# ynotstartups/implisolid

Hardware: AMD Instinct MI355X
Metric: Mvoxels/s (eval+MC) at 256^3 & 512^3 (higher is better)
Workload: dtype f32; 1 GPU; config4: seeded ~20-node MP5 CSG tree with twist/union/difference (scenes.config4, seed 20251015), box [-1,1]^3, R=512, eval+MC, mesh resident in HBM; resolution=512, voxels=134217728, samples=135005697, cells=135796744, verts=360248, faces=720496, program_instr=42, tree_depth=8, parallelism=zslab1, voxels_per_rank=134217728

## Files before the change

### implisolid_amd/csrc/abi.hip

```cpp
#include <chrono>
#include <cmath>
#include <cstdio>
#include <cstdlib>
#include <cstring>
#include <ctime>
#include <map>
#include <memory>
#include <string>
#include <vector>
#include <thread>
#include <mutex>
#include <algorithm>
#include <functional>

#include "../../include/implisolid.h"
#include "engine.hpp"
#include "batch_device.hpp"
#include "brick_modes.hpp"
#include "jit.hpp"

#include <chrono>
#include <rocprofiler-sdk-roctx/roctx.h>
#include "host.hpp"
#include "ob02.hpp"
// ... 1381 lines not shown
#define SLAB_TRY(expr)                                 \
    try {                                              \
        expr;                                          \
    } catch (const std::exception& e) {                \
        report(e.what(), false);                       \
        return -1;                                     \
    }                                                  \
    return 0;

int implisolid_slab_eval(implisolid_slab* s, void* stream) { SLAB_TRY(s->engine.eval_field((hipStream_t)stream)) }
int implisolid_slab_count(implisolid_slab* s, void* stream) { SLAB_TRY(s->engine.count((hipStream_t)stream)) }
int implisolid_slab_emit(implisolid_slab* s, const uint32_t* d_offsets, void* stream) {
    SLAB_TRY(s->engine.emit(d_offsets, (hipStream_t)stream))
}
int implisolid_slab_emit_verts(implisolid_slab* s, void* stream) {
    SLAB_TRY(s->engine.emit_verts((hipStream_t)stream))
}
int implisolid_slab_emit_faces(implisolid_slab* s, const uint32_t* d_offsets, const uint32_t* d_gathered, int rank,
                               void* stream) {
    SLAB_TRY(s->engine.emit_faces(d_offsets, d_gathered, rank, (hipStream_t)stream))
}
const uint32_t* implisolid_slab_counters(implisolid_slab* s) { return s->engine.d_counters(); }
int implisolid_slab_counts(implisolid_slab* s, void* stream, uint32_t out[3]) {
    try {
        bool of = false;
        SlabCounts c = s->engine.read_counts((hipStream_t)stream, &of);
        const bool grew = s->engine.ensure_capacity(c);
        out[0] = c.n_verts();
        out[1] = c.n_faces();
        out[2] = (of || grew) ? 1u : 0u;
    } catch (const std::exception& e) {
        report(e.what(), false);
        return -1;
    }
    return 0;
}
int implisolid_slab_grid(implisolid_slab* s, int32_t out[8]) {
    const GridDesc& g = s->engine.grid();
    const int32_t v[8] = {g.R, g.res, g.cz0, g.cz1, g.cz_emit, g.fz0, g.fz1, s->engine.depth()};
    std::memcpy(out, v, sizeof v);
    return 0;
}
int implisolid_slab_copy_counts(implisolid_slab* s, uint32_t* d_dst, void* stream) {
    SLAB_TRY(IMPLI_HIP(hipMemcpyAsync(d_dst, s->engine.d_counters() + 2, 4 * sizeof(uint32_t), hipMemcpyDeviceToDevice,
                                      (hipStream_t)stream)))
}
int implisolid_slab_copy_mesh(implisolid_slab* s, float* d_verts, int32_t* d_faces, int64_t nv, int64_t nf, void* stream) {
    SLAB_TRY(
        if (nv > 0) IMPLI_HIP(hipMemcpyAsync(d_verts, s->engine.d_verts(), (size_t)nv * 12, hipMemcpyDeviceToDevice, (hipStream_t)stream));
        if (nf > 0) IMPLI_HIP(hipMemcpyAsync(d_faces, s->engine.d_faces(), (size_t)nf * 12, hipMemcpyDeviceToDevice, (hipStream_t)stream)))
}
int implisolid_slab_set_offsets(implisolid_slab* s, uint32_t voff, uint32_t foff) {
    SLAB_TRY(s->engine.set_offsets(voff, foff))
}
int implisolid_slab_download(implisolid_slab* s, float* verts, int32_t* faces, void* stream) {
    try {
        bool of = false;
        const SlabCounts c = s->engine.read_counts((hipStream_t)stream, &of);
        if (of) throw HipError("slab output overflowed; call implisolid_slab_counts and emit again");
        s->engine.download(verts, faces, c, (hipStream_t)stream);
    } catch (const std::exception& e) {
        report(e.what(), false);
        return -1;
    }
    return 0;
}
int implisolid_slab_emit_normals(implisolid_slab* s, void* stream) { SLAB_TRY(s->engine.emit_normals((hipStream_t)stream)) }
float* implisolid_slab_normals(implisolid_slab* s) { return s->engine.d_normals(); }
int implisolid_slab_download_normals(implisolid_slab* s, float* out, void* stream) {
    try {
        const SlabCounts c = s->engine.read_counts((hipStream_t)stream, nullptr);
        s->engine.download_normals(out, c, (hipStream_t)stream);
    } catch (const std::exception& e) {
        report(e.what(), false);
        return -1;
    }
    return 0;
}
float* implisolid_slab_verts(implisolid_slab* s) { return s->engine.d_verts(); }
int32_t* implisolid_slab_faces(implisolid_slab* s) { return s->engine.d_faces(); }
float* implisolid_slab_field(implisolid_slab* s) { return s->engine.d_field(); }

int implisolid_slab_stats_n(implisolid_slab* s, int64_t* out, int n) {
    constexpr int kStats = 10;
    try {
        if (!out || n < 0) throw InputError("slab_stats: null output or negative length");
        uint32_t c[16];
        s->engine.raw_counters(c, 0);
        const GridDesc& g = s->engine.grid();
        const int64_t v[kStats] = {
            n_units(g),
            c[6],
            c[2], c[3], c[4], c[5],
            g.n_cells,
            c[14],
            c[1],
            c[0]};
        for (int k = 0; k < n && k < kStats; ++k) out[k] = v[k];
        return kStats;
    } catch (const std::exception& e) {
        report(e.what(), false);
        return -1;
    }
}

int implisolid_slab_stats(implisolid_slab* s, int64_t out[8]) {
    return implisolid_slab_stats_n(s, out, 8) < 0 ? -1 : 0;
}

int implisolid_slab_used_jit(implisolid_slab* s) { return s->engine.used_baked() ? 2 : s->engine.used_jit() ? 1 : 0; }
void implisolid_set_jit(int mode) { TreeJit::instance().set_mode(mode); }
void implisolid_set_jit_bake(int mode) { TreeJit::instance().set_bake(mode); }
void implisolid_jit_wait(void) { TreeJit::instance().wait_idle(); }
void implisolid_jit_stats(int32_t out[4], double* compile_seconds) {
    TreeJit& j = TreeJit::instance();
    out[0] = j.mode();
    out[1] = j.bake();
    out[2] = j.compiled();
    out[3] = j.disk_hits();
    if (compile_seconds) *compile_seconds = j.compile_seconds();
}
void implisolid_set_jit_max_modules(int n) { TreeJit::instance().set_max_modules(n); }
void implisolid_jit_modules(int32_t out[3]) {
    TreeJit& j = TreeJit::instance();
    out[0] = j.modules();
    out[1] = j.max_modules();
    out[2] = j.evicted();
}

int implisolid_slab_set_timing(implisolid_slab* s, int on) { SLAB_TRY(s->engine.set_timing(on != 0)) }
int implisolid_slab_kernel_times(implisolid_slab* s, float ms[6]) { SLAB_TRY(s->engine.kernel_times(ms)) }
int implisolid_slab_kernel_times_each(implisolid_slab* s, float ms[8]) { SLAB_TRY(s->engine.kernel_times_each(ms)) }

int64_t implisolid_slab_read_signs(implisolid_slab* s, uint8_t* out, int64_t capacity) {
    try {
        const GridDesc& g = s->engine.grid();
        const int64_t rows = (int64_t)g.n * (g.fz1 - g.fz0), rw = sign_row_words(g);
        const int64_t n = rows * g.n;
        if (out) {
            if (capacity < n) throw InputError("implisolid_slab_read_signs: buffer too small");
            std::vector<uint64_t> w((size_t)(rows * rw));
            IMPLI_HIP(hipDeviceSynchronize());
            IMPLI_HIP(hipMemcpy(w.data(), s->engine.d_signs(), w.size() * sizeof(uint64_t), hipMemcpyDeviceToHost));
            for (int64_t r = 0; r < rows; ++r)
                for (int x = 0; x < g.n; ++x) out[r * g.n + x] = (uint8_t)((w[(size_t)(r * rw + x / 64)] >> (x % 64)) & 1u);
        }
        return n;
    } catch (const std::exception& e) {
        report(e.what(), false);
        return -1;
    }
}

int implisolid_slab_brick_stats(implisolid_slab* s, int64_t out[3]) {
    try {
        s->engine.brick_stats(out, 0);
    } catch (const std::exception& e) {
        report(e.what(), false);
        return -1;
    }
    return 0;
}

int64_t implisolid_slab_read_field(implisolid_slab* s, float* out, int64_t capacity) {
    try {
        const GridDesc& g = s->engine.grid();
        const int64_t n = (int64_t)g.n * g.n * (int64_t)(g.fz1 - g.fz0);
        if (out) {
            if (capacity < n) throw InputError("implisolid_slab_read_field: buffer too small");
            IMPLI_HIP(hipDeviceSynchronize());
            std::vector<float> raw((size_t)field_samples(g));
            if (!raw.empty())
                IMPLI_HIP(hipMemcpy(raw.data(), s->engine.d_field(), raw.size() * sizeof(float), hipMemcpyDeviceToHost));
            const int layers = g.fz1 - g.fz0;
            for (int l = 0; l < layers; ++l)
                for (int y = 0; y < g.n; ++y)
                    for (int x = 0; x < g.n; ++x)
                        out[((int64_t)l * g.n + y) * g.n + x] = raw[(size_t)field_index(g, x, y, l)];
        }
// ... 585 lines not shown
```

### implisolid_amd/csrc/mc.hip

```cpp
#include <algorithm>
#include <cstdlib>
#include <stdexcept>

#include "eval_bricks.hpp"
#include "ifunc_device.hpp"
#include "kernels.hpp"
#include "mc_device.hpp"
#include "batch_device.hpp"

namespace impli {

GridDesc make_grid(int R, const float box[6], int cz0, int cz1, int cz_emit) {
    GridDesc g{};
    g.R = R;
    g.res = R + 5;
    g.n = R + 3;
    g.m = R + 2;
    for (int a = 0; a < 3; ++a) {
        const float width = box[2 * a + 1] - box[2 * a];
        g.w[a] = width / (float)R;
        g.lo[a] = box[2 * a];
        g.i0[a] = box[2 * a] / g.w[a] - 2.f;
    }
    g.cz0 = cz0;
// ... 12 lines not shown
        int n = 0;
        for (; s[n]; ++n) c.tri[n] = (uint8_t)((s[n] <= '9') ? s[n] - '0' : s[n] - 'a' + 10);
        c.ntri = (uint8_t)(n / 3);
        c.rank[0] = c.rank[1] = c.rank[2] = -1;
        int r = 0;
        for (int k = 0; k < n; ++k) {
            const int e = c.tri[k];
            const int slot = (e == 5) ? 0 : (e == 6) ? 1 : (e == 10) ? 2 : -1;
            if (slot >= 0 && c.rank[slot] < 0) c.rank[slot] = (int8_t)r++;
        }
        c.nown = (uint8_t)r;
        static const int owner_of_edge[12] = {5, 4, 4, 6, 2, 0, 0, 1, 3, 2, 0, 1};
        for (int k = 0; k < n; ++k) c.owners = (uint8_t)(c.owners | (1u << owner_of_edge[c.tri[k]]));
        auto neg = [ci](int k) { return (ci >> k) & 1; };
        const int crossing = (neg(5) ^ neg(6)) + (neg(6) ^ neg(7)) + (neg(2) ^ neg(6));
        int ec = 0, ei = 0, v = 0, ff = 0, opp = 0;
        for (const auto& e : kCubeEdges) { ec += neg(e[0]) ^ neg(e[1]); ei += neg(e[0]) & neg(e[1]); }
        for (int k = 0; k < 8; ++k) v += neg(k);
        for (const auto& f : kCubeFaces) ff += neg(f[0]) & neg(f[1]) & neg(f[2]) & neg(f[3]);
        for (const auto& o : kCubeOpposite) opp += (v == 6 && !neg(o[0]) && !neg(o[1])) ? 1 : 0;
        const int ntri_formula = (ci == 0 || ci == 255) ? 0 : ec - 2 * (v - ei + ff + 2 * opp);
        if (crossing != c.nown || (c.ntri > 0) != (ci != 0 && ci != 255) || ntri_formula != c.ntri)
            throw std::runtime_error("marching cubes: case table violates the count kernel's assumptions");
        out[ci] = c;
    }
}

namespace {

__device__ __forceinline__ uint32_t wave_sum(uint32_t x) {
#pragma unroll
    for (int o = 32; o > 0; o >>= 1) x += __shfl_xor(x, o, 64);
    return x;
}

__device__ __forceinline__ void mc_count_body(const GridDesc& g, const MCBuffers& b) {
    __shared__ uint32_t s_u[kGroupUnits][4];
    __shared__ uint32_t s_cm[kGroupUnits];
    __shared__ uint16_t s_fp[kGroupUnits * kMaxChunks];
    __shared__ uint32_t s_nf;
    const int t = threadIdx.x, nt_ = blockDim.x;
    for (int k = t; k < 4 * kGroupUnits; k += nt_) (&s_u[0][0])[k] = 0u;
    for (int k = t; k < kGroupUnits; k += nt_) s_cm[k] = 0u;
    if (t == 0) s_nf = 0u;
    const int64_t G = blockIdx.x;
    const int nch = n_chunks(g);
    const int64_t rows = n_rows(g), nu = n_units(g);
    const int64_t row0 = G * kGroupUnits * kUnitRows;
    __syncthreads();
    for (int p0 = 0; p0 < kGroupUnits * nch; p0 += nt_) {
        const int p = p0 + t, ui = p / nch, c = p - ui * nch;
        const int64_t u = G * kGroupUnits + ui;
        const bool cand = p < kGroupUnits * nch && u < nu && (!b.umark || b.umark[u * nch + c] == b.mark_id);
        const uint64_t m = __ballot(cand);
        uint32_t base = 0;
        if ((t & 63) == 0 && m) base = atomicAdd(&s_nf, (uint32_t)__popcll((unsigned long long)m));
        base = __shfl(base, 0, 64);
        if (cand) s_fp[base + __popcll((unsigned long long)(m & ((1ull << (t & 63)) - 1ull)))] = (uint16_t)(ui * kMaxChunks + c);
    }
    __syncthreads();
    const int n_items = (int)s_nf * kUnitRows;
    for (int i = t; i < n_items; i += nt_) {
        ChunkBits k;
        const uint32_t pr = s_fp[i / kUnitRows];
        const int ui = (int)(pr / kMaxChunks), c = (int)(pr % kMaxChunks);
        const int rb = ui * kUnitRows + i % kUnitRows;
        const bool ok = row0 + rb < rows;
        load_chunk(g, b.signs, ok ? row0 + rb : 0, c, k);
        if (!ok) k.nt = 0;
        if (!k.nt) continue;
        if (c < kChunkMaskBits) atomicOr(&s_cm[ui], 1u << c);
        const unsigned own = (unsigned)(__popcll((unsigned long long)((k.t01 ^ k.t11) & k.nt)) +
                                        __popcll((unsigned long long)((k.s11 ^ k.t11) & k.nt)) +
                                        __popcll((unsigned long long)((k.t10 ^ k.t11) & k.nt)));
        unsigned tri = 0, act = 0, hal = 0;
        if (k.z >= g.cz_emit) {
            act = (unsigned)__popcll((unsigned long long)k.nt);
            tri = chunk_triangles(k);
        } else {
            hal = own;
        }
        uint32_t* d = s_u[ui];
        if (own) atomicAdd(&d[0], own);
        if (tri) { atomicAdd(&d[1], tri); atomicAdd(&d[2], act); }
        if (hal) atomicAdd(&d[3], hal);
    }
    __syncthreads();
    if (t < 64) {
        const int64_t u = G * kGroupUnits + t;
        const uint32_t own = s_u[t][0], tri = s_u[t][1], act = s_u[t][2], hal = s_u[t][3];
        const bool ne = u < nu && (own | tri) != 0;
        const uint32_t eo = wave_incl_scan<uint32_t>(own, t) - own;
        const uint32_t et = wave_incl_scan<uint32_t>(tri, t) - tri;
        const uint32_t ea = wave_incl_scan<uint32_t>(act, t) - act;
        const uint64_t m = __ballot(ne);
        const uint32_t pos = (uint32_t)__popcll((unsigned long long)(m & ((1ull << t) - 1ull)));
        const uint32_t parts = ne ? min((uint32_t)kMaxParts, max(1u, (act + kPartCells - 1) / kPartCells)) : 0u;
        const bool heavy = act > kHeavyCells;
        const uint32_t ph = heavy ? parts : 0u, pl = heavy ? 0u : parts;
        const uint32_t eph = wave_incl_scan<uint32_t>(ph, t) - ph, epl = wave_incl_scan<uint32_t>(pl, t) - pl;
        if (ne) {
            b.unit_cnt[G * kGroupUnits + pos] = make_uint4((uint32_t)t, eo, et, ea);
            b.unit_part[G * kGroupUnits + pos] = (heavy ? eph : epl) | (parts << 16) | ((uint32_t)heavy << 20);
            b.unit_cmask[G * kGroupUnits + pos] = s_cm[t];
        }
        const uint32_t sums[kScanParts + 1] = {__shfl(eo + own, 63, 64), __shfl(et + tri, 63, 64),
                                               __shfl(ea + act, 63, 64), wave_sum(hal), __shfl(eph + ph, 63, 64),
                                               __shfl(epl + pl, 63, 64), (uint32_t)__popcll((unsigned long long)m)};
        if (t <= kScanParts) {
            const uint32_t v = t == 0 ? sums[0] : t == 1 ? sums[1] : t == 2 ? sums[2] : t == 3 ? sums[3]
                             : t == 4 ? sums[4] : t == 5 ? sums[5] : sums[6];
            b.scan_blk[(int64_t)t * gridDim.x + G] = v;
        }
    }
}
__global__ __launch_bounds__(512) void k_mc_count(GridDesc g, MCBuffers b) { mc_count_body(g, b); }

constexpr int kScanBlock = 256;
constexpr int kScanRows = kScanParts + 1;
template <int BS = kScanBlock>
__device__ __forceinline__ void unit_scan_body(const GridDesc& g, const MCBuffers& b) {
    static_assert(BS >= kGroupUnits, "a lane per unit of the group");
    __shared__ uint32_t s_part[BS / 64][kScanRows];
    __shared__ uint32_t s_base[kScanRows];
    const int64_t G = blockIdx.x, ng = n_groups(g);
    const int t = threadIdx.x, lane = t & 63, wid = t >> 6;
    const bool last = G == ng - 1;
    const uint32_t nne = b.scan_blk[kScanParts * ng + G];
    if (nne == 0 && !last) return;
    const uint4 e = b.unit_cnt[G * kGroupUnits + (t < (int)nne ? t : 0)];
    const uint32_t pp = b.unit_part[G * kGroupUnits + (t < (int)nne ? t : 0)];
    const uint32_t cm = b.unit_cmask[G * kGroupUnits + (t < (int)nne ? t : 0)];
    uint32_t acc[kScanRows] = {0u, 0u, 0u, 0u, 0u, 0u, 0u};
#pragma unroll 4
    for (int64_t i = t; i < G; i += BS)
#pragma unroll
        for (int c = 0; c < kScanRows; ++c) acc[c] += b.scan_blk[c * ng + i];
#pragma unroll
    for (int c = 0; c < kScanRows; ++c) {
        const uint32_t s = wave_sum(acc[c]);
        if (lane == 0) s_part[wid][c] = s;
    }
    __syncthreads();
    if (t < kScanRows) {
        uint32_t s = 0;
#pragma unroll
        for (int w = 0; w < BS / 64; ++w) s += s_part[w][t];
        s_base[t] = s;
    }
    __syncthreads();
    if (t < (int)nne) {
        const uint4 ent = make_uint4((uint32_t)(G * kGroupUnits) + e.x, s_base[0] + e.y, s_base[1] + e.z, s_base[2] + e.w);
        const uint32_t P = (pp >> 16) & 15u;
        const bool heavy = (pp >> 20) & 1u;
        const uint32_t r = (heavy ? s_base[4] : s_base[5]) + (pp & 0xffffu);
        for (uint32_t q = 0; q < P; ++q) {
            const uint32_t at = heavy ? r + q : b.cap_parts - 1u - (r + q);
            b.ulist[at] = ent;
            b.upart[at] = q | (P << 4) | (cm << 8);
        }
    }
    if (last && t == 0) {
        const uint32_t nh = s_base[4] + b.scan_blk[4 * ng + G];
        b.counters[7] = nh;
        b.counters[0] = nh + s_base[5] + b.scan_blk[5 * ng + G];
        b.counters[1] = s_base[3] + b.scan_blk[3 * ng + G];
        b.counters[2] = s_base[0] + b.scan_blk[G];
        b.counters[3] = s_base[1] + b.scan_blk[ng + G];
        b.counters[4] = s_base[2] + b.scan_blk[2 * ng + G];
        b.counters[5] = s_base[3] + b.scan_blk[3 * ng + G];
        b.counters[6] = s_base[6] + nne;
    }
}
__global__ __launch_bounds__(kScanBlock) void k_unit_scan(GridDesc g, MCBuffers b) { unit_scan_body<>(g, b); }

__global__ __launch_bounds__(64 * kVertsWaves) __attribute__((amdgpu_waves_per_eu(6))) void k_mc_cells(const CaseInfo* __restrict__ cases, GridDesc g, MCBuffers b) {
    mc_cells_body(cases, g, b);
}

constexpr unsigned kFacesBlocks = 2048;
static_assert(kFacesBlocks % 8 == 0, "k_mc_faces' XCD remap needs a multiple of 8 blocks");

__constant__ uint8_t c_edge_owner_idx[12] = {5, 4, 4, 6, 2, 0, 0, 1, 3, 2, 0, 1};
__constant__ uint8_t c_edge_slot[12] = {1, 0, 1, 0, 1, 0, 1, 0, 2, 2, 2, 2};

__device__ __forceinline__ void face_record(const CaseInfo* s_case, uint32_t (*s_w)[256], const GridDesc& g,
                                            const MCBuffers& b, uint32_t Voff, uint32_t i) {
    const int t = threadIdx.x;
    const uint4 r = b.records[i];
    const uint32_t L = r.x, ci = r.y, fbase = r.z;
    const CaseInfo& C = s_case[ci];
    const int ntri = C.ntri;
    if (fbase + ntri > (uint64_t)b.cap_f) { *b.overflow = 1u; return; }
    const uint32_t need = C.owners;
    const uint32_t m = (uint32_t)g.m, m2 = m * m;
    const uint32_t d[6] = {1u, m, m + 1u, m2, m2 + m, m2 + 1u};
    const IdTriple* vid = reinterpret_cast<const IdTriple*>(b.vid);
    IdTriple w[7];
    w[0] = vid[L];
#pragma unroll
    for (int q = 0; q < 6; ++q) w[q + 1] = vid[((need >> (q + 1)) & 1u) ? L - d[q] : L];
#pragma unroll
    for (int e = 0; e < 12; ++e) {
        const IdTriple& q = w[c_edge_owner_idx[e]];
        const int sl = c_edge_slot[e];
        s_w[e][t] = sl == 0 ? q.a : sl == 1 ? q.b : q.c;
    }
    int32_t* out = b.faces + 3 * (size_t)fbase;
    for (int k = 0; k < ntri; ++k) {
        IdTriple f;
        f.a = Voff + s_w[C.tri[3 * k]][t];
        f.b = Voff + s_w[C.tri[3 * k + 1]][t];
        f.c = Voff + s_w[C.tri[3 * k + 2]][t];
        *reinterpret_cast<IdTriple*>(out + 3 * k) = f;
    }
}

__device__ __forceinline__ void mc_faces_body(const CaseInfo* __restrict__ cases, const GridDesc& g, const MCBuffers& b) {
    __shared__ CaseInfo s_case[256];
    __shared__ uint32_t s_w[12][256];
    const int t = threadIdx.x;
    s_case[t] = cases[t];
    __syncthreads();
    const uint32_t n_rec = b.counters[4];
    const uint32_t lim = n_rec < (uint64_t)b.cap_rec ? n_rec : (uint32_t)b.cap_rec;
    uint32_t Voff = b.offsets ? b.offsets[0] : 0u;
    if (b.gathered)
        for (int r = 0; r < b.rank; ++r) Voff += b.gathered[4 * r] - b.gathered[4 * r + 3];
    const uint32_t nb = gridDim.x, lb = (blockIdx.x % 8u) * (nb / 8u) + blockIdx.x / 8u;
    const uint32_t per = (lim + nb - 1u) / nb, i_end = min(lim, (lb + 1u) * per);
    for (uint32_t i = lb * per + t; i < i_end; i += 256) face_record(s_case, s_w, g, b, Voff, i);
}

__global__ __launch_bounds__(256) void k_mc_faces(const CaseInfo* __restrict__ cases, GridDesc g, MCBuffers b) {
    mc_faces_body(cases, g, b);
}

__global__ __launch_bounds__(512) void k_mc_count_b(const ObjArgs* __restrict__ objs, GridDesc g) {
    mc_count_body(g, objs[blockIdx.y].mc);
}
template <int B>
__global__ __launch_bounds__(B) void k_unit_scan_b(const ObjArgs* __restrict__ objs, GridDesc g) {
    unit_scan_body<B>(g, objs[blockIdx.y].mc);
}
__global__ __launch_bounds__(64 * kVertsWaves) void k_mc_cells_b(const CaseInfo* __restrict__ cases,
                                                                const ObjArgs* __restrict__ objs, int n, GridDesc g) {
    __shared__ uint32_t s_cw[256];
    __shared__ uint64_t s_bits[kVertsWaves][9][64];
    __shared__ uint32_t s_excl[kVertsWaves][64];
    __shared__ uint32_t s_pre[kMaxBatchObjects + 4];
    const int t = threadIdx.x, wid = t >> 6;
    for (int k = t; k < 256; k += blockDim.x) s_cw[k] = case_word(cases[k]);
    const uint32_t total = batch_prefix(objs, n, 0, 1u, 0xffffffffu, s_pre);
    for (uint32_t e = blockIdx.x * kVertsWaves + wid; e < total; e += gridDim.x * kVertsWaves) {
        const int k = __builtin_amdgcn_readfirstlane(batch_object_of(s_pre, n, e));
        mc_cells_part(s_cw, g, objs[k].mc, e - s_pre[k], s_bits[wid], s_excl[wid]);
    }
}
__global__ __launch_bounds__(256) void k_gather_counters(const ObjArgs* __restrict__ objs, int n, uint32_t* __restrict__ out) {
    const int i = blockIdx.x * 256 + threadIdx.x;
    if (i < n * kCounterWords) out[i] = objs[i / kCounterWords].counters[i % kCounterWords];
}
__global__ __launch_bounds__(256) void k_zero_pieces(const ZeroPiece* __restrict__ pieces) {
    const ZeroPiece z = pieces[blockIdx.x];
    uint8_t* p = reinterpret_cast<uint8_t*>(z.p);
    const uint32_t n16 = z.n / 16;
    for (uint32_t i = threadIdx.x; i < n16; i += 256) reinterpret_cast<uint4*>(p)[i] = uint4{0, 0, 0, 0};
    for (uint32_t i = n16 * 16 + threadIdx.x; i < z.n; i += 256) p[i] = 0;
}
__global__ __launch_bounds__(256) void k_mc_faces_b(const CaseInfo* __restrict__ cases, const ObjArgs* __restrict__ objs,
                                                    int n, GridDesc g) {
    __shared__ CaseInfo s_case[256];
    __shared__ uint32_t s_w[12][256];
    __shared__ uint32_t s_pre[kMaxBatchObjects + 4];
    const int t = threadIdx.x;
    s_case[t] = cases[t];
    const uint32_t total = batch_prefix(objs, n, 4, 1u, 0xffffffffu, s_pre);
    for (uint32_t gi = blockIdx.x * 256 + t; gi < total; gi += gridDim.x * 256) {
        const int k = batch_object_of(s_pre, n, gi);
        const MCBuffers& b = objs[k].mc;
        const uint32_t i = gi - s_pre[k];
        if (i >= (uint64_t)b.cap_rec) { *b.overflow = 1u; continue; }
        face_record(s_case, s_w, g, b, b.offsets ? b.offsets[0] : 0u, i);
    }
}

}

void launch_mc_count(const CaseInfo* d_cases, const GridDesc& g, const MCBuffers& b, hipStream_t s) {
    const int64_t ng = n_groups(g);
    if (ng == 0) return;
    const int items = kGroupUnits * kUnitRows * ((g.m + 63) / 64);
    const unsigned threads = (unsigned)std::min(512, (items + 63) / 64 * 64);
    (void)d_cases;
    k_mc_count<<<(unsigned)ng, threads, 0, s>>>(g, b);
}

void launch_mc_scan(const GridDesc& g, const MCBuffers& b, hipStream_t s) {
    const int64_t ng = n_groups(g);
    if (ng > 0) k_unit_scan<<<(unsigned)ng, kScanBlock, 0, s>>>(g, b);
}

void launch_mc_faces(const CaseInfo* d_cases, const GridDesc& g, const MCBuffers& b, hipStream_t s) {
    k_mc_faces<<<kFacesBlocks, 256, 0, s>>>(d_cases, g, b);
}

void launch_mc_verts(const CaseInfo* d_cases, const GridDesc& g, const MCBuffers& b, hipStream_t s) {
    const int64_t nu = n_units(g);
    if (nu > 0) {
        k_mc_cells<<<(unsigned)std::min<int64_t>((nu + kVertsWaves - 1) / kVertsWaves, kVertsMaxBlocks),
                     64 * kVertsWaves, 0, s>>>(d_cases, g, b);
    }
}

}

namespace impli {

constexpr unsigned kBatchCellBlocks = 4096, kBatchFaceBlocks = 2048;
constexpr int kBatchCountLanes = 128;

void launch_gather_counters(const ObjArgs* d_objs, int n, uint32_t* d_out, hipStream_t s) {
    if (n > 0) k_gather_counters<<<(unsigned)((n * kCounterWords + 255) / 256), 256, 0, s>>>(d_objs, n, d_out);
}

void launch_zero_pieces(const ZeroPiece* d_pieces, int n, hipStream_t s) {
    if (n > 0) k_zero_pieces<<<(unsigned)n, 256, 0, s>>>(d_pieces);
}

void launch_batch_mc(const ObjArgs* d_objs, int n, const CaseInfo* d_cases, const GridDesc& g, hipStream_t s) {
    const int64_t ng = n_groups(g), nu = n_units(g);
    if (ng == 0 || n <= 0) return;
    const int items = kGroupUnits * kUnitRows * ((g.m + 63) / 64);
    const unsigned threads = (unsigned)std::min(kBatchCountLanes, (items + 63) / 64 * 64);
    k_mc_count_b<<<dim3((unsigned)ng, (unsigned)n), threads, 0, s>>>(d_objs, g);
    if (ng <= 64) k_unit_scan_b<64><<<dim3((unsigned)ng, (unsigned)n), 64, 0, s>>>(d_objs, g);
    else k_unit_scan_b<kScanBlock><<<dim3((unsigned)ng, (unsigned)n), kScanBlock, 0, s>>>(d_objs, g);
    (void)nu;
    k_mc_cells_b<<<kBatchCellBlocks, 64 * kVertsWaves, 0, s>>>(d_cases, d_objs, n, g);
// ... 5 lines not shown
```

### implisolid_amd/csrc/mc_device.hpp

```cpp
#pragma once
#include "eval_bricks.hpp"
#include "mc_types.hpp"

namespace impli {

template <typename T>
__device__ __forceinline__ T wave_incl_scan(T x, int lane) {
#pragma unroll
    for (int o = 1; o < 64; o <<= 1) {
        const T y = __shfl_up(x, o, 64);
        if (lane >= o) x += y;
    }
    return x;
}

struct __attribute__((packed, aligned(4))) IdTriple { uint32_t a, b, c; };

struct ChunkBits {
    uint64_t s00, t00, s10, t10, s01, t01, s11, t11, nt;
    int y, z, x0;
};

__device__ __forceinline__ void load_chunk(const GridDesc& g, const uint64_t* __restrict__ signs, int64_t row, int c,
                                           ChunkBits& k) {
    const int rw = sign_row_words(g);
    const int r32 = (int)row;
    k.y = r32 % g.m + 1;
    k.z = r32 / g.m + g.cz0;
    k.x0 = 64 * c + 1;
    const int64_t r00 = ((int64_t)(k.z - g.fz0) * g.n + (k.y - 1)) * rw;
    const int64_t rows[4] = {r00, r00 + rw, r00 + (int64_t)g.n * rw, r00 + (int64_t)g.n * rw + rw};
    uint64_t w[4], nx[4], s[4], t[4];
#pragma unroll
    for (int q = 0; q < 4; ++q) {
        w[q] = signs[rows[q] + c];
        nx[q] = signs[rows[q] + c + 1];
    }
    const uint64_t keep = 0ull - (uint64_t)(c + 1 < rw);
#pragma unroll
    for (int q = 0; q < 4; ++q) {
        s[q] = w[q];
        t[q] = (w[q] >> 1) | ((nx[q] & keep) << 63);
    }
    k.s00 = s[0]; k.t00 = t[0]; k.s10 = s[1]; k.t10 = t[1]; k.s01 = s[2]; k.t01 = t[2]; k.s11 = s[3]; k.t11 = t[3];
    const uint64_t all = s[0] & t[0] & s[1] & t[1] & s[2] & t[2] & s[3] & t[3];
    const uint64_t any = s[0] | t[0] | s[1] | t[1] | s[2] | t[2] | s[3] | t[3];
    const int left = g.m - 64 * c;
    const uint64_t valid = left >= 64 ? ~0ull : ((1ull << left) - 1ull);
    k.nt = any & ~all & valid;
}

constexpr int kCubeEdges[12][2] = {{0, 1}, {1, 2}, {2, 3}, {3, 0}, {4, 5}, {5, 6},
                                   {6, 7}, {7, 4}, {0, 4}, {1, 5}, {2, 6}, {3, 7}};
constexpr int kCubeFaces[6][4] = {{0, 1, 2, 3}, {4, 5, 6, 7}, {0, 1, 5, 4}, {1, 2, 6, 5}, {2, 3, 7, 6}, {3, 0, 4, 7}};
constexpr int kCubeOpposite[4][2] = {{0, 6}, {1, 7}, {2, 4}, {3, 5}};

__device__ __forceinline__ unsigned chunk_triangles(const ChunkBits& k) {
    const uint64_t c[8] = {k.s00, k.t00, k.t10, k.s10, k.s01, k.t01, k.t11, k.s11};
    const uint64_t nt = k.nt;
    int ec = 0, ei = 0, v = 0, ff = 0, opp = 0;
#pragma unroll
    for (int e = 0; e < 12; ++e) {
        const uint64_t a = c[kCubeEdges[e][0]], b = c[kCubeEdges[e][1]];
        ec += __popcll((unsigned long long)((a ^ b) & nt));
        ei += __popcll((unsigned long long)(a & b & nt));
    }
#pragma unroll
    for (int q = 0; q < 8; ++q) v += __popcll((unsigned long long)(c[q] & nt));
#pragma unroll
    for (int f = 0; f < 6; ++f)
        ff += __popcll((unsigned long long)(c[kCubeFaces[f][0]] & c[kCubeFaces[f][1]] & c[kCubeFaces[f][2]] &
                                            c[kCubeFaces[f][3]] & nt));
#pragma unroll
    for (int o = 0; o < 4; ++o) {
        const int a = kCubeOpposite[o][0], b = kCubeOpposite[o][1];
        uint64_t rest = ~c[a] & ~c[b] & nt;
#pragma unroll
        for (int q = 0; q < 8; ++q)
            if (q != a && q != b) rest &= c[q];
        opp += __popcll((unsigned long long)rest);
    }
    return (unsigned)(ec - 2 * (v - ei + ff + 2 * opp));
}

__device__ __forceinline__ unsigned chunk_ci(const ChunkBits& k, int j) {
    return (unsigned)((k.s00 >> j) & 1u) | ((unsigned)((k.t00 >> j) & 1u) << 1) | ((unsigned)((k.s10 >> j) & 1u) << 3) |
           ((unsigned)((k.t10 >> j) & 1u) << 2) | ((unsigned)((k.s01 >> j) & 1u) << 4) |
           ((unsigned)((k.t01 >> j) & 1u) << 5) | ((unsigned)((k.s11 >> j) & 1u) << 7) |
           ((unsigned)((k.t11 >> j) & 1u) << 6);
}

constexpr int kPackShift[3] = {0, 8, 18};
constexpr unsigned kPackMask[3] = {0xffu, 0x3ffu, 0x7fu};
__device__ __forceinline__ unsigned pack3(unsigned own, unsigned tri, unsigned act) {
    return own | (tri << 8) | (act << 18);
}
__device__ __forceinline__ unsigned fld(unsigned p, int i) { return (p >> kPackShift[i]) & kPackMask[i]; }

__device__ __forceinline__ int select_bit(uint64_t x, uint32_t r) {
    int pos = 0;
#pragma unroll
    for (int w = 32; w > 0; w >>= 1) {
        const uint32_t c = (uint32_t)__popcll((unsigned long long)(x & ((1ull << w) - 1ull)));
        if (r >= c) { r -= c; x >>= w; pos += w; }
    }
    return pos;
}

__device__ __forceinline__ uint32_t case_word(const CaseInfo& c) {
    uint32_t w = (uint32_t)c.nown | ((uint32_t)c.ntri << 2);
    for (int s = 0; s < 3; ++s) w |= (uint32_t)(c.rank[s] + 1) << (5 + 3 * s);
    return w;
}

__device__ __forceinline__ void mc_cells_part(const uint32_t* s_cw, const GridDesc& g, const MCBuffers& b, uint32_t e,
                                              uint64_t (*bits)[64], uint32_t* excl) {
    const int lane = threadIdx.x & 63;
    const uint32_t H = b.counters[1];
    const int nch = (g.m + 63) / 64;
    const int64_t rows = n_rows(g);
    const int items = kUnitRows * nch;
    {
        const uint32_t nh = b.counters[7];
        e = e < nh ? e : b.cap_parts - 1u - (e - nh);
        const uint4 ent = b.ulist[e];
        const uint32_t up = b.upart[e];
        const uint32_t part = up & 15u, parts = (up >> 4) & 15u;
        const uint32_t cmask = nch <= kChunkMaskBits ? up >> 8 : ~0u;
        const int64_t u = ent.x;
        uint32_t vrun0 = ent.y, frun0 = ent.z, arun0 = ent.w;
        uint32_t win = 0;
        for (int i0 = 0; i0 < items; i0 += 64) {
            const int i = i0 + lane;
            ChunkBits k;
            k.nt = 0;
            k.z = 0;
            const int64_t irow = u * kUnitRows + i / nch;
            const int ic = i % nch;
            if (i < items) {
                if (irow < rows && (ic >= kChunkMaskBits || ((cmask >> ic) & 1u))) load_chunk(g, b.signs, irow, ic, k);
            }
            const uint32_t cnt = (uint32_t)__popcll((unsigned long long)k.nt);
            const uint32_t incl = wave_incl_scan<uint32_t>(cnt, lane);
            const uint32_t total = __shfl(incl, 63, 64);
            __builtin_amdgcn_wave_barrier();
            bits[0][lane] = k.s00; bits[1][lane] = k.t00; bits[2][lane] = k.s10; bits[3][lane] = k.t10;
            bits[4][lane] = k.s01; bits[5][lane] = k.t01; bits[6][lane] = k.s11; bits[7][lane] = k.t11;
            bits[8][lane] = k.nt;
            excl[lane] = incl - cnt;
            __builtin_amdgcn_wave_barrier();
            for (uint32_t e0 = 0; e0 < total; e0 += 64, ++win) {
                const bool mine = win % parts == part;
                const uint32_t ce = e0 + (uint32_t)lane;
                const bool has = ce < total;
                int q = 0;
#pragma unroll
                for (int step = 32; step > 0; step >>= 1)
                    if (excl[q + step] <= ce) q += step;
                const int j = has ? select_bit(bits[8][q], ce - excl[q]) : 0;
                const unsigned ci =
                    has ? (unsigned)((bits[0][q] >> j) & 1u) | ((unsigned)((bits[1][q] >> j) & 1u) << 1) |
                              ((unsigned)((bits[3][q] >> j) & 1u) << 2) | ((unsigned)((bits[2][q] >> j) & 1u) << 3) |
                              ((unsigned)((bits[4][q] >> j) & 1u) << 4) | ((unsigned)((bits[5][q] >> j) & 1u) << 5) |
                              ((unsigned)((bits[7][q] >> j) & 1u) << 6) | ((unsigned)((bits[6][q] >> j) & 1u) << 7)
                        : 0u;
                const int it = i0 + q;
                const int64_t erow = u * kUnitRows + it / nch;
                const int x = 64 * (it % nch) + 1 + j;
                const int z = (int)erow / g.m + g.cz0;
                const uint32_t L = (uint32_t)(erow * g.m + (x - 1));
                const uint32_t cw = s_cw[ci];
                const unsigned c_nown = cw & 3u, c_ntri = (cw >> 2) & 7u;
                const bool emit = has && z >= g.cz_emit;
                const unsigned own = has ? c_nown : 0u, tri = emit ? c_ntri : 0u, act = (emit && c_ntri) ? 1u : 0u;
                const unsigned p = pack3(own, tri, act);
                const unsigned inc = wave_incl_scan<unsigned>(p, lane);
                const unsigned pre = inc - p, tot = __shfl(inc, 63, 64);
                const uint32_t vrun = vrun0 + fld(pre, 0);
                if (mine) {
                    const int y = (int)erow % g.m + 1;
                    const int sx = x - 1, sy = y - 1, sl = z - g.fz0;
                    const int cx = has ? sx : 0, cy = has ? sy : 0, cl = has ? sl : 0, d = has ? 1 : 0;
                    const uint32_t fx0 = field_x_term(cx), fx1 = field_x_term(cx + d);
                    const uint32_t fy0 = field_y_term(g, cy), fy1 = field_y_term(g, cy + d);
                    const int64_t fl0 = field_layer_term(g, cl), fl1 = field_layer_term(g, cl + d);
                    const float r7 = b.field[fl1 + (fy1 + fx1)];
                    const float r5 = b.field[fl1 + (fy0 + fx1)];
                    const float r6 = b.field[fl1 + (fy1 + fx0)];
                    const float r3 = b.field[fl0 + (fy1 + fx1)];
                    const bool sx1 = sealed_xy(g, sx + 1), sy1 = sealed_xy(g, sy + 1), sz1 = sealed_z(g, sl + 1);
                    const bool sx0 = sealed_xy(g, sx), sy0 = sealed_xy(g, sy), sz0 = sealed_z(g, sl);
                    const float f7 = (sx1 || sy1 || sz1) ? kSealed : r7;
                    const float f5 = (sx1 || sy0 || sz1) ? kSealed : r5;
                    const float f6 = (sx0 || sy1 || sz1) ? kSealed : r6;
                    const float f3 = (sx1 || sy1 || sz0) ? kSealed : r3;
                    uint32_t ids[3];
#pragma unroll
                    for (int slot = 0; slot < 3; ++slot) ids[slot] = vrun + (uint32_t)((cw >> (5 + 3 * slot)) & 7u) - 1u - H;
                    if (has && own) {
                        const float fx = ((float)x + g.i0[0]) * g.w[0];
                        const float fy = ((float)y + g.i0[1]) * g.w[1];
                        const float fz = ((float)z + g.i0[2]) * g.w[2];
                        const float fx2 = fx + g.w[0], fy2 = fy + g.w[1], fz2 = fz + g.w[2];
#pragma unroll
                        for (int slot = 0; slot < 3; ++slot) {
                            const int r = (int)((cw >> (5 + 3 * slot)) & 7u) - 1;
                            if (r < 0 || !emit) continue;
                            const uint32_t out = ids[slot];
                            if (out >= (uint64_t)b.cap_v) { *b.overflow = 1u; continue; }
                            float px, py, pz;
                            if (slot == 0) { const float mu = (0.f - f5) / (f7 - f5); px = fx2; py = fy + mu * g.w[1]; pz = fz2; }
                            else if (slot == 1) { const float mu = (0.f - f6) / (f7 - f6); px = fx + mu * g.w[0]; py = fy2; pz = fz2; }
                            else { const float mu = (0.f - f3) / (f7 - f3); px = fx2; py = fy2; pz = fz + mu * g.w[2]; }
                            b.verts[3 * (size_t)out] = px; b.verts[3 * (size_t)out + 1] = py; b.verts[3 * (size_t)out + 2] = pz;
                        }
                        *reinterpret_cast<IdTriple*>(b.vid + (size_t)L * 3) = IdTriple{ids[0], ids[1], ids[2]};
                    }
                    if (act) {
                        const uint32_t arun = arun0 + fld(pre, 2);
                        if (arun < (uint64_t)b.cap_rec) b.records[arun] = make_uint4(L, ci, frun0 + fld(pre, 1), (uint32_t)erow);
                        else *b.overflow = 1u;
                    }
                }
                vrun0 += fld(tot, 0);
                frun0 += fld(tot, 1);
                arun0 += fld(tot, 2);
            }
        }
    }
}

__device__ __forceinline__ void mc_cells_body(const CaseInfo* __restrict__ cases, const GridDesc& g, const MCBuffers& b) {
    __shared__ uint32_t s_cw[256];
    __shared__ uint64_t s_bits[kVertsWaves][9][64];
    __shared__ uint32_t s_excl[kVertsWaves][64];
    const int t = threadIdx.x, wid = t >> 6;
    const uint32_t n_ne = b.counters[0];
    const uint32_t w0 = blockIdx.x * kVertsWaves;
    if (w0 >= n_ne) return;
    for (int k = t; k < 256; k += blockDim.x) s_cw[k] = case_word(cases[k]);
    __syncthreads();
    for (uint32_t e = w0 + wid; e < n_ne; e += gridDim.x * kVertsWaves) mc_cells_part(s_cw, g, b, e, s_bits[wid], s_excl[wid]);
}

}
```

### implisolid_amd/csrc/mc_types.hpp

```cpp
#pragma once
#include "grid.hpp"
#include "program.hpp"

namespace impli {

struct CaseInfo {
    uint8_t ntri;
    uint8_t nown;
    int8_t rank[3];
    uint8_t pad;
    uint8_t tri[15];
    uint8_t owners;
    uint8_t pad2[10];
};
static_assert(sizeof(CaseInfo) == 32, "CaseInfo layout");
constexpr int kUnitRows = 4;
constexpr int kGroupUnits = 64;
constexpr int kVertsWaves = 4;
constexpr int kVertsMaxBlocks = 4096;
constexpr int kScanParts = 6;
constexpr uint32_t kHeavyCells = 64;
constexpr int kPartCells = 128;
constexpr int kMaxParts = 8;
constexpr int kChunkMaskBits = 24;
struct MCBuffers {
    const float* field;
    const uint64_t* signs;
    uint4* unit_cnt;
    uint32_t* unit_part;
    uint32_t* unit_cmask;
    uint32_t* scan_blk;
    uint4* ulist;
    uint32_t* upart;
    uint32_t cap_parts;
    const uint32_t* umark;
    uint32_t mark_id;
    uint32_t* counters;
    uint32_t* vid;
    uint4* records;
    float* verts;
    int32_t* faces;
    int64_t cap_v, cap_f, cap_rec;
    const uint32_t* offsets;
    const uint32_t* gathered;
    int rank;
    uint32_t* overflow;
};
__host__ __device__ inline int64_t n_rows(const GridDesc& g) { return (int64_t)g.m * (g.cz1 - g.cz0); }
__host__ __device__ inline int64_t n_units(const GridDesc& g) { return (n_rows(g) + kUnitRows - 1) / kUnitRows; }
__host__ __device__ inline int64_t n_groups(const GridDesc& g) { return (n_units(g) + kGroupUnits - 1) / kGroupUnits; }
__host__ __device__ inline int n_chunks(const GridDesc& g) { return (g.m + 63) / 64; }
constexpr int kMaxChunks = 128;

}
```

Before: 1.364 million Mvoxels/s.

## Pack two small MC units into one wave using half-wave processing

Units with at most 32 non-trivial cells and a small chunk mask are classified as 'small' in the count/scan stages. They are placed in interleaved slots of the part list so that two of them are processed by one 64-lane wave, one per 32-lane half, in a new pair path. This cuts the number of wave work items in the cell-emission kernel, which reduces wave-level overhead on sparse surface units. In exchange it adds a classification bit, an extra scan row, a more complex slot indexing scheme and a new code path to maintain.

```diff
diff --git a/implisolid_amd/csrc/abi.hip b/implisolid_amd/csrc/abi.hip
--- a/implisolid_amd/csrc/abi.hip
+++ b/implisolid_amd/csrc/abi.hip
@@ -1487,7 +1487,7 @@
 float* implisolid_slab_field(implisolid_slab* s) { return s->engine.d_field(); }
 
 int implisolid_slab_stats_n(implisolid_slab* s, int64_t* out, int n) {
-    constexpr int kStats = 10;
+    constexpr int kStats = 13;
     try {
         if (!out || n < 0) throw InputError("slab_stats: null output or negative length");
         uint32_t c[16];
@@ -1500,6 +1500,9 @@
             g.n_cells,
             c[14],
             c[1],
+            (int64_t)c[0] + c[8] / 2,
+            c[8],
+            c[7],
             c[0]};
         for (int k = 0; k < n && k < kStats; ++k) out[k] = v[k];
         return kStats;
diff --git a/implisolid_amd/csrc/mc.hip b/implisolid_amd/csrc/mc.hip
--- a/implisolid_amd/csrc/mc.hip
+++ b/implisolid_amd/csrc/mc.hip
@@ -118,13 +118,14 @@
         }
         uint32_t* d = s_u[ui];
         if (own) atomicAdd(&d[0], own);
-        if (tri) { atomicAdd(&d[1], tri); atomicAdd(&d[2], act); }
+        if (tri) atomicAdd(&d[1], tri);
+        atomicAdd(&d[2], act | ((uint32_t)__popcll((unsigned long long)k.nt) << 16));
         if (hal) atomicAdd(&d[3], hal);
     }
     __syncthreads();
     if (t < 64) {
         const int64_t u = G * kGroupUnits + t;
-        const uint32_t own = s_u[t][0], tri = s_u[t][1], act = s_u[t][2], hal = s_u[t][3];
+        const uint32_t own = s_u[t][0], tri = s_u[t][1], act = s_u[t][2] & 0xffffu, ntc = s_u[t][2] >> 16, hal = s_u[t][3];
         const bool ne = u < nu && (own | tri) != 0;
         const uint32_t eo = wave_incl_scan<uint32_t>(own, t) - own;
         const uint32_t et = wave_incl_scan<uint32_t>(tri, t) - tri;
@@ -133,19 +134,25 @@
         const uint32_t pos = (uint32_t)__popcll((unsigned long long)(m & ((1ull << t) - 1ull)));
         const uint32_t parts = ne ? min((uint32_t)kMaxParts, max(1u, (act + kPartCells - 1) / kPartCells)) : 0u;
         const bool heavy = act > kHeavyCells;
-        const uint32_t ph = heavy ? parts : 0u, pl = heavy ? 0u : parts;
+        const bool small = ne && ntc <= kPairCells && nch <= kChunkMaskBits &&
+                           (uint32_t)(kUnitRows * __popc(s_cm[t])) <= kPairCells;
+        const uint32_t ph = heavy ? parts : 0u, pl = (heavy || small) ? 0u : parts, ps = small ? 1u : 0u;
         const uint32_t eph = wave_incl_scan<uint32_t>(ph, t) - ph, epl = wave_incl_scan<uint32_t>(pl, t) - pl;
+        const uint64_t msm = __ballot(small);
+        const uint32_t eps = (uint32_t)__popcll((unsigned long long)(msm & ((1ull << t) - 1ull)));
         if (ne) {
             b.unit_cnt[G * kGroupUnits + pos] = make_uint4((uint32_t)t, eo, et, ea);
-            b.unit_part[G * kGroupUnits + pos] = (heavy ? eph : epl) | (parts << 16) | ((uint32_t)heavy << 20);
+            b.unit_part[G * kGroupUnits + pos] =
+                (heavy ? eph : small ? eps : epl) | (parts << 16) | ((uint32_t)heavy << 20) | (ps << 21);
             b.unit_cmask[G * kGroupUnits + pos] = s_cm[t];
         }
         const uint32_t sums[kScanParts + 1] = {__shfl(eo + own, 63, 64), __shfl(et + tri, 63, 64),
                                                __shfl(ea + act, 63, 64), wave_sum(hal), __shfl(eph + ph, 63, 64),
-                                               __shfl(epl + pl, 63, 64), (uint32_t)__popcll((unsigned long long)m)};
+                                               __shfl(epl + pl, 63, 64), (uint32_t)__popcll((unsigned long long)msm),
+                                               (uint32_t)__popcll((unsigned long long)m)};
         if (t <= kScanParts) {
             const uint32_t v = t == 0 ? sums[0] : t == 1 ? sums[1] : t == 2 ? sums[2] : t == 3 ? sums[3]
-                             : t == 4 ? sums[4] : t == 5 ? sums[5] : sums[6];
+                             : t == 4 ? sums[4] : t == 5 ? sums[5] : t == 6 ? sums[6] : sums[7];
             b.scan_blk[(int64_t)t * gridDim.x + G] = v;
         }
     }
@@ -167,7 +174,7 @@
     const uint4 e = b.unit_cnt[G * kGroupUnits + (t < (int)nne ? t : 0)];
     const uint32_t pp = b.unit_part[G * kGroupUnits + (t < (int)nne ? t : 0)];
     const uint32_t cm = b.unit_cmask[G * kGroupUnits + (t < (int)nne ? t : 0)];
-    uint32_t acc[kScanRows] = {0u, 0u, 0u, 0u, 0u, 0u, 0u};
+    uint32_t acc[kScanRows] = {0u, 0u, 0u, 0u, 0u, 0u, 0u, 0u};
 #pragma unroll 4
     for (int64_t i = t; i < G; i += BS)
 #pragma unroll
@@ -188,24 +195,26 @@
     if (t < (int)nne) {
         const uint4 ent = make_uint4((uint32_t)(G * kGroupUnits) + e.x, s_base[0] + e.y, s_base[1] + e.z, s_base[2] + e.w);
         const uint32_t P = (pp >> 16) & 15u;
-        const bool heavy = (pp >> 20) & 1u;
-        const uint32_t r = (heavy ? s_base[4] : s_base[5]) + (pp & 0xffffu);
+        const bool heavy = (pp >> 20) & 1u, small = (pp >> 21) & 1u;
+        const uint32_t r = (heavy ? s_base[4] : small ? s_base[6] : s_base[5]) + (pp & 0xffffu);
         for (uint32_t q = 0; q < P; ++q) {
-            const uint32_t at = heavy ? r + q : b.cap_parts - 1u - (r + q);
+            const uint32_t at = heavy ? r + q : b.cap_parts - (small ? 2u : 1u) - 2u * (r + q);
             b.ulist[at] = ent;
             b.upart[at] = q | (P << 4) | (cm << 8);
         }
     }
     if (last && t == 0) {
         const uint32_t nh = s_base[4] + b.scan_blk[4 * ng + G];
+        const uint32_t ns = s_base[6] + b.scan_blk[6 * ng + G];
         b.counters[7] = nh;
-        b.counters[0] = nh + s_base[5] + b.scan_blk[5 * ng + G];
+        b.counters[8] = ns;
+        b.counters[0] = nh + (ns + 1u) / 2u + s_base[5] + b.scan_blk[5 * ng + G];
         b.counters[1] = s_base[3] + b.scan_blk[3 * ng + G];
         b.counters[2] = s_base[0] + b.scan_blk[G];
         b.counters[3] = s_base[1] + b.scan_blk[ng + G];
         b.counters[4] = s_base[2] + b.scan_blk[2 * ng + G];
         b.counters[5] = s_base[3] + b.scan_blk[3 * ng + G];
-        b.counters[6] = s_base[6] + nne;
+        b.counters[6] = s_base[7] + nne;
     }
 }
 __global__ __launch_bounds__(kScanBlock) void k_unit_scan(GridDesc g, MCBuffers b) { unit_scan_body<>(g, b); }
@@ -290,7 +299,7 @@
     const uint32_t total = batch_prefix(objs, n, 0, 1u, 0xffffffffu, s_pre);
     for (uint32_t e = blockIdx.x * kVertsWaves + wid; e < total; e += gridDim.x * kVertsWaves) {
         const int k = __builtin_amdgcn_readfirstlane(batch_object_of(s_pre, n, e));
-        mc_cells_part(s_cw, g, objs[k].mc, e - s_pre[k], s_bits[wid], s_excl[wid]);
+        mc_cells_item(s_cw, g, objs[k].mc, e - s_pre[k], s_bits[wid], s_excl[wid]);
     }
 }
 __global__ __launch_bounds__(256) void k_gather_counters(const ObjArgs* __restrict__ objs, int n, uint32_t* __restrict__ out) {
diff --git a/implisolid_amd/csrc/mc_device.hpp b/implisolid_amd/csrc/mc_device.hpp
--- a/implisolid_amd/csrc/mc_device.hpp
+++ b/implisolid_amd/csrc/mc_device.hpp
@@ -4,11 +4,11 @@
 
 namespace impli {
 
-template <typename T>
+template <typename T, int W = 64>
 __device__ __forceinline__ T wave_incl_scan(T x, int lane) {
 #pragma unroll
-    for (int o = 1; o < 64; o <<= 1) {
-        const T y = __shfl_up(x, o, 64);
+    for (int o = 1; o < W; o <<= 1) {
+        const T y = __shfl_up(x, o, W);
         if (lane >= o) x += y;
     }
     return x;
@@ -107,13 +107,77 @@
     return pos;
 }
 
+__device__ __forceinline__ int select_bit32(uint32_t x, uint32_t r) {
+    int pos = 0;
+#pragma unroll
+    for (int w = 16; w > 0; w >>= 1) {
+        const uint32_t c = (uint32_t)__popc(x & ((1u << w) - 1u));
+        if (r >= c) { r -= c; x >>= w; pos += w; }
+    }
+    return pos;
+}
+
 __device__ __forceinline__ uint32_t case_word(const CaseInfo& c) {
     uint32_t w = (uint32_t)c.nown | ((uint32_t)c.ntri << 2);
     for (int s = 0; s < 3; ++s) w |= (uint32_t)(c.rank[s] + 1) << (5 + 3 * s);
     return w;
 }
 
-__device__ __forceinline__ void mc_cells_part(const uint32_t* s_cw, const GridDesc& g, const MCBuffers& b, uint32_t e,
+__device__ __forceinline__ void cell_emit(const GridDesc& g, const MCBuffers& b, uint32_t H, bool has, bool emit,
+                                          int64_t erow, int x, int z, uint32_t L, unsigned ci, uint32_t cw, unsigned own,
+                                          unsigned act, uint32_t vrun, uint32_t frun, uint32_t arun) {
+    const int y = (int)erow % g.m + 1;
+    const int sx = x - 1, sy = y - 1, sl = z - g.fz0;
+    const int cx = has ? sx : 0, cy = has ? sy : 0, cl = has ? sl : 0, d = has ? 1 : 0;
+    const uint32_t fx0 = field_x_term(cx), fx1 = field_x_term(cx + d);
+    const uint32_t fy0 = field_y_term(g, cy), fy1 = field_y_term(g, cy + d);
+    const int64_t fl0 = field_layer_term(g, cl), fl1 = field_layer_term(g, cl + d);
+    const float r7 = b.field[fl1 + (fy1 + fx1)];
+    const float r5 = b.field[fl1 + (fy0 + fx1)];
+    const float r6 = b.field[fl1 + (fy1 + fx0)];
+    const float r3 = b.field[fl0 + (fy1 + fx1)];
+    const bool sx1 = sealed_xy(g, sx + 1), sy1 = sealed_xy(g, sy + 1), sz1 = sealed_z(g, sl + 1);
+    const bool sx0 = sealed_xy(g, sx), sy0 = sealed_xy(g, sy), sz0 = sealed_z(g, sl);
+    const float f7 = (sx1 || sy1 || sz1) ? kSealed : r7;
+    const float f5 = (sx1 || sy0 || sz1) ? kSealed : r5;
+    const float f6 = (sx0 || sy1 || sz1) ? kSealed : r6;
+    const float f3 = (sx1 || sy1 || sz0) ? kSealed : r3;
+    uint32_t ids[3];
+#pragma unroll
+    for (int slot = 0; slot < 3; ++slot) ids[slot] = vrun + (uint32_t)((cw >> (5 + 3 * slot)) & 7u) - 1u - H;
+    if (has && own) {
+        const float fx = ((float)x + g.i0[0]) * g.w[0];
+        const float fy = ((float)y + g.i0[1]) * g.w[1];
+        const float fz = ((float)z + g.i0[2]) * g.w[2];
+        const float fx2 = fx + g.w[0], fy2 = fy + g.w[1], fz2 = fz + g.w[2];
+#pragma unroll
+        for (int slot = 0; slot < 3; ++slot) {
+            const int r = (int)((cw >> (5 + 3 * slot)) & 7u) - 1;
+            if (r < 0 || !emit) continue;
+            const uint32_t out = ids[slot];
+            if (out >= (uint64_t)b.cap_v) { *b.overflow = 1u; continue; }
+            float px, py, pz;
+            if (slot == 0) { const float mu = (0.f - f5) / (f7 - f5); px = fx2; py = fy + mu * g.w[1]; pz = fz2; }
+            else if (slot == 1) { const float mu = (0.f - f6) / (f7 - f6); px = fx + mu * g.w[0]; py = fy2; pz = fz2; }
+            else { const float mu = (0.f - f3) / (f7 - f3); px = fx2; py = fy2; pz = fz + mu * g.w[2]; }
+            b.verts[3 * (size_t)out] = px; b.verts[3 * (size_t)out + 1] = py; b.verts[3 * (size_t)out + 2] = pz;
+        }
+        *reinterpret_cast<IdTriple*>(b.vid + (size_t)L * 3) = IdTriple{ids[0], ids[1], ids[2]};
+    }
+    if (act) {
+        if (arun < (uint64_t)b.cap_rec) b.records[arun] = make_uint4(L, ci, frun, (uint32_t)erow);
+        else *b.overflow = 1u;
+    }
+}
+
+__device__ __forceinline__ unsigned staged_ci(const uint64_t (*bits)[64], int q, int j) {
+    return (unsigned)((bits[0][q] >> j) & 1u) | ((unsigned)((bits[1][q] >> j) & 1u) << 1) |
+           ((unsigned)((bits[3][q] >> j) & 1u) << 2) | ((unsigned)((bits[2][q] >> j) & 1u) << 3) |
+           ((unsigned)((bits[4][q] >> j) & 1u) << 4) | ((unsigned)((bits[5][q] >> j) & 1u) << 5) |
+           ((unsigned)((bits[7][q] >> j) & 1u) << 6) | ((unsigned)((bits[6][q] >> j) & 1u) << 7);
+}
+
+__device__ __forceinline__ void mc_cells_part(const uint32_t* s_cw, const GridDesc& g, const MCBuffers& b, uint32_t at,
                                               uint64_t (*bits)[64], uint32_t* excl) {
     const int lane = threadIdx.x & 63;
     const uint32_t H = b.counters[1];
@@ -121,10 +185,8 @@
     const int64_t rows = n_rows(g);
     const int items = kUnitRows * nch;
     {
-        const uint32_t nh = b.counters[7];
-        e = e < nh ? e : b.cap_parts - 1u - (e - nh);
-        const uint4 ent = b.ulist[e];
-        const uint32_t up = b.upart[e];
+        const uint4 ent = b.ulist[at];
+        const uint32_t up = b.upart[at];
         const uint32_t part = up & 15u, parts = (up >> 4) & 15u;
         const uint32_t cmask = nch <= kChunkMaskBits ? up >> 8 : ~0u;
         const int64_t u = ent.x;
@@ -158,12 +220,7 @@
                 for (int step = 32; step > 0; step >>= 1)
                     if (excl[q + step] <= ce) q += step;
                 const int j = has ? select_bit(bits[8][q], ce - excl[q]) : 0;
-                const unsigned ci =
-                    has ? (unsigned)((bits[0][q] >> j) & 1u) | ((unsigned)((bits[1][q] >> j) & 1u) << 1) |
-                              ((unsigned)((bits[3][q] >> j) & 1u) << 2) | ((unsigned)((bits[2][q] >> j) & 1u) << 3) |
-                              ((unsigned)((bits[4][q] >> j) & 1u) << 4) | ((unsigned)((bits[5][q] >> j) & 1u) << 5) |
-                              ((unsigned)((bits[7][q] >> j) & 1u) << 6) | ((unsigned)((bits[6][q] >> j) & 1u) << 7)
-                        : 0u;
+                const unsigned ci = has ? staged_ci(bits, q, j) : 0u;
                 const int it = i0 + q;
                 const int64_t erow = u * kUnitRows + it / nch;
                 const int x = 64 * (it % nch) + 1 + j;
@@ -177,57 +234,75 @@
                 const unsigned inc = wave_incl_scan<unsigned>(p, lane);
                 const unsigned pre = inc - p, tot = __shfl(inc, 63, 64);
                 const uint32_t vrun = vrun0 + fld(pre, 0);
-                if (mine) {
-                    const int y = (int)erow % g.m + 1;
-                    const int sx = x - 1, sy = y - 1, sl = z - g.fz0;
-                    const int cx = has ? sx : 0, cy = has ? sy : 0, cl = has ? sl : 0, d = has ? 1 : 0;
-                    const uint32_t fx0 = field_x_term(cx), fx1 = field_x_term(cx + d);
-                    const uint32_t fy0 = field_y_term(g, cy), fy1 = field_y_term(g, cy + d);
-                    const int64_t fl0 = field_layer_term(g, cl), fl1 = field_layer_term(g, cl + d);
-                    const float r7 = b.field[fl1 + (fy1 + fx1)];
-                    const float r5 = b.field[fl1 + (fy0 + fx1)];
-                    const float r6 = b.field[fl1 + (fy1 + fx0)];
-                    const float r3 = b.field[fl0 + (fy1 + fx1)];
-                    const bool sx1 = sealed_xy(g, sx + 1), sy1 = sealed_xy(g, sy + 1), sz1 = sealed_z(g, sl + 1);
-                    const bool sx0 = sealed_xy(g, sx), sy0 = sealed_xy(g, sy), sz0 = sealed_z(g, sl);
-                    const float f7 = (sx1 || sy1 || sz1) ? kSealed : r7;
-                    const float f5 = (sx1 || sy0 || sz1) ? kSealed : r5;
-                    const float f6 = (sx0 || sy1 || sz1) ? kSealed : r6;
-                    const float f3 = (sx1 || sy1 || sz0) ? kSealed : r3;
-                    uint32_t ids[3];
-#pragma unroll
-                    for (int slot = 0; slot < 3; ++slot) ids[slot] = vrun + (uint32_t)((cw >> (5 + 3 * slot)) & 7u) - 1u - H;
-                    if (has && own) {
-                        const float fx = ((float)x + g.i0[0]) * g.w[0];
-                        const float fy = ((float)y + g.i0[1]) * g.w[1];
-                        const float fz = ((float)z + g.i0[2]) * g.w[2];
-                        const float fx2 = fx + g.w[0], fy2 = fy + g.w[1], fz2 = fz + g.w[2];
-#pragma unroll
-                        for (int slot = 0; slot < 3; ++slot) {
-                            const int r = (int)((cw >> (5 + 3 * slot)) & 7u) - 1;
-                            if (r < 0 || !emit) continue;
-                            const uint32_t out = ids[slot];
-                            if (out >= (uint64_t)b.cap_v) { *b.overflow = 1u; continue; }
-                            float px, py, pz;
-                            if (slot == 0) { const float mu = (0.f - f5) / (f7 - f5); px = fx2; py = fy + mu * g.w[1]; pz = fz2; }
-                            else if (slot == 1) { const float mu = (0.f - f6) / (f7 - f6); px = fx + mu * g.w[0]; py = fy2; pz = fz2; }
-                            else { const float mu = (0.f - f3) / (f7 - f3); px = fx2; py = fy2; pz = fz + mu * g.w[2]; }
-                            b.verts[3 * (size_t)out] = px; b.verts[3 * (size_t)out + 1] = py; b.verts[3 * (size_t)out + 2] = pz;
-                        }
-                        *reinterpret_cast<IdTriple*>(b.vid + (size_t)L * 3) = IdTriple{ids[0], ids[1], ids[2]};
-                    }
-                    if (act) {
-                        const uint32_t arun = arun0 + fld(pre, 2);
-                        if (arun < (uint64_t)b.cap_rec) b.records[arun] = make_uint4(L, ci, frun0 + fld(pre, 1), (uint32_t)erow);
-                        else *b.overflow = 1u;
-                    }
-                }
+                if (mine)
+                    cell_emit(g, b, H, has, emit, erow, x, z, L, ci, cw, own, act, vrun, frun0 + fld(pre, 1),
+                              arun0 + fld(pre, 2));
                 vrun0 += fld(tot, 0);
                 frun0 += fld(tot, 1);
                 arun0 += fld(tot, 2);
             }
         }
     }
+}
+
+__device__ __forceinline__ void mc_cells_pair(const uint32_t* s_cw, const GridDesc& g, const MCBuffers& b, uint32_t p,
+                                              uint32_t ns, uint64_t (*bits)[64], uint32_t* excl) {
+    int lane = threadIdx.x & 63;
+    asm volatile("" : "+v"(lane));
+    const int hl = lane & 31, hb = lane & 32;
+    const uint32_t H = b.counters[1];
+    const int64_t rows = n_rows(g);
+    const uint32_t k = 2u * p + (uint32_t)(lane >> 5);
+    const bool live = k < ns;
+    const uint32_t at = b.cap_parts - 2u - 2u * (live ? k : k - 1u);
+    const uint4 ent = b.ulist[at];
+    const uint32_t cmask = b.upart[at] >> 8;
+    const int nc = max(1, (int)__popc(cmask));
+    const uint32_t u = ent.x;
+    const int ir = (int)(((uint32_t)hl * ((uint32_t)((0x1F242A333F557FFFull >> (8 * (nc - 1))) & 0xffu) + 1u)) >> 8);
+    const uint32_t irow = u * kUnitRows + (uint32_t)ir;
+    const bool item = live && cmask != 0u && ir < kUnitRows && (int64_t)irow < rows;
+    const int ic = select_bit32(cmask, (uint32_t)(hl - ir * nc));
+    ChunkBits kb;
+    load_chunk(g, b.signs, item ? (int64_t)irow : 0, item ? ic : 0, kb);
+    if (!item) kb.nt = 0;
+    const uint32_t cnt = (uint32_t)__popcll((unsigned long long)kb.nt);
+    const uint32_t incl = wave_incl_scan<uint32_t, 32>(cnt, hl);
+    const uint32_t total = __shfl(incl, 31, 32);
+    __builtin_amdgcn_wave_barrier();
+    bits[0][lane] = kb.s00; bits[1][lane] = kb.t00; bits[2][lane] = kb.s10; bits[3][lane] = kb.t10;
+    bits[4][lane] = kb.s01; bits[5][lane] = kb.t01; bits[6][lane] = kb.s11; bits[7][lane] = kb.t11;
+    bits[8][lane] = kb.nt;
+    excl[lane] = (incl - cnt) | ((uint32_t)ic << 8) | ((uint32_t)ir << 16);
+    __builtin_amdgcn_wave_barrier();
+    const uint32_t ce = (uint32_t)hl;
+    const bool has = ce < total;
+    int q = 0;
+#pragma unroll
+    for (int step = 16; step > 0; step >>= 1)
+        if ((excl[hb + q + step] & 0xffu) <= ce) q += step;
+    const uint32_t qw = excl[hb + q];
+    const int j = has ? select_bit(bits[8][hb + q], ce - (qw & 0xffu)) : 0;
+    const unsigned ci = has ? staged_ci(bits, hb + q, j) : 0u;
+    const int64_t erow = (int64_t)(u * kUnitRows + (qw >> 16));
+    const int x = 64 * (int)((qw >> 8) & 0xffu) + 1 + j;
+    const int z = (int)erow / g.m + g.cz0;
+    const uint32_t L = (uint32_t)(erow * g.m + (x - 1));
+    const uint32_t cw = s_cw[ci];
+    const unsigned c_nown = cw & 3u, c_ntri = (cw >> 2) & 7u;
+    const bool emit = has && z >= g.cz_emit;
+    const unsigned own = has ? c_nown : 0u, tri = emit ? c_ntri : 0u, act = (emit && c_ntri) ? 1u : 0u;
+    const unsigned pk = pack3(own, tri, act);
+    const unsigned pre = wave_incl_scan<unsigned, 32>(pk, hl) - pk;
+    cell_emit(g, b, H, has, emit, erow, x, z, L, ci, cw, own, act, ent.y + fld(pre, 0), ent.z + fld(pre, 1),
+              ent.w + fld(pre, 2));
+}
+
+__device__ __forceinline__ void mc_cells_item(const uint32_t* s_cw, const GridDesc& g, const MCBuffers& b, uint32_t e,
+                                              uint64_t (*bits)[64], uint32_t* excl) {
+    const uint32_t nh = b.counters[7], ns = b.counters[8], np = (ns + 1u) / 2u;
+    if (e >= nh && e - nh < np) mc_cells_pair(s_cw, g, b, e - nh, ns, bits, excl);
+    else mc_cells_part(s_cw, g, b, e < nh ? e : b.cap_parts - 1u - 2u * (e - nh - np), bits, excl);
 }
 
 __device__ __forceinline__ void mc_cells_body(const CaseInfo* __restrict__ cases, const GridDesc& g, const MCBuffers& b) {
@@ -240,7 +315,7 @@
     if (w0 >= n_ne) return;
     for (int k = t; k < 256; k += blockDim.x) s_cw[k] = case_word(cases[k]);
     __syncthreads();
-    for (uint32_t e = w0 + wid; e < n_ne; e += gridDim.x * kVertsWaves) mc_cells_part(s_cw, g, b, e, s_bits[wid], s_excl[wid]);
-}
-
-}
+    for (uint32_t e = w0 + wid; e < n_ne; e += gridDim.x * kVertsWaves) mc_cells_item(s_cw, g, b, e, s_bits[wid], s_excl[wid]);
+}
+
+}
diff --git a/implisolid_amd/csrc/mc_types.hpp b/implisolid_amd/csrc/mc_types.hpp
--- a/implisolid_amd/csrc/mc_types.hpp
+++ b/implisolid_amd/csrc/mc_types.hpp
@@ -18,8 +18,9 @@
 constexpr int kGroupUnits = 64;
 constexpr int kVertsWaves = 4;
 constexpr int kVertsMaxBlocks = 4096;
-constexpr int kScanParts = 6;
+constexpr int kScanParts = 7;
 constexpr uint32_t kHeavyCells = 64;
+constexpr uint32_t kPairCells = 32;
 constexpr int kPartCells = 128;
 constexpr int kMaxParts = 8;
 constexpr int kChunkMaskBits = 24;
```

Result: faster. 1.381 million Mvoxels/s, median of 6 (+1.2%).
